# Chemical118/TREW

Hardware: AMD Instinct MI355X
Metric: Gbases/s scanned (short 5 32, 150 bp reads) (higher is better)
Workload: dtype u32

## Files before the change

include/trew_hip.h:

```cpp
#ifndef TREW_HIP_H
#define TREW_HIP_H

#include <stddef.h>
#include <stdint.h>

#ifdef __cplusplus
extern "C" {
#endif

#define TREW_HIP_ABI_VERSION 4

enum {
    TREW_MODE_SHORT = 0,
    TREW_MODE_PAIR = 1,
    TREW_MODE_LONG = 2,
    TREW_MODE_SEGMENT = 3
};

enum {
    TREW_TABLE_FORWARD_HIGH = 0,
    TREW_TABLE_FORWARD_LOW = 1,
    TREW_TABLE_BACKWARD_HIGH = 2,
    TREW_TABLE_BACKWARD_LOW = 3,
    TREW_TABLE_BOTH_HIGH = 4,
    TREW_TABLE_BOTH_LOW = 5,
    TREW_NUM_TABLES = 6
};

enum {
    TREW_FLAG_NO_FILTER = 1,
    TREW_FLAG_DEBUG_NO_EMIT = 2,
    TREW_FLAG_DEBUG_NO_KLOOP = 4,
    TREW_FLAG_DEBUG_POISON_LDS = 32,
    TREW_FLAG_DEBUG_WIDE_NO_WAIT = 128,
    TREW_FLAG_NO_TIMING = 64,
    TREW_FLAG_COMPAT_G1 = 512,
    TREW_FLAG_DEBUG_NO_JOINT = 2048,
    TREW_FLAG_DEBUG_NO_UNI_DRAIN = 4096,
    TREW_FLAG_DEBUG_NO_GROUP = 1024,
    TREW_FLAG_DEBUG_ANNOT_GENERAL = 8192,
    TREW_FLAG_TRACK_PRESSURE = 256
};

typedef struct {
    int32_t min_mer;
    int32_t max_mer;
    double low_baseline;
    double high_baseline;
    int32_t slice_length;
    int32_t mode;
    int32_t device;
    int32_t n_slots;
    uint64_t max_batch_words;
    uint64_t max_batch_reads;
    uint32_t table_log2_slots;
    uint32_t flags;
    uint64_t max_batch_ascii_bytes;
} trew_hip_params;

typedef struct {
    const uint32_t *words;
// ... 116 lines not shown
```

trew_amd/__init__.py:

```python
from . import capi
from .capi import (
    FLAG_NO_FILTER,
    FLAG_DEBUG_ANNOT_GENERAL,
    FLAG_DEBUG_POISON_LDS,
    FLAG_NO_TIMING,
    FLAG_TRACK_PRESSURE,
    FLAG_COMPAT_G1,
    FLAG_DEBUG_NO_GROUP,
    FLAG_DEBUG_NO_JOINT,
    FLAG_DEBUG_NO_UNI_DRAIN,
    FLAG_DEBUG_WIDE_NO_WAIT,
    MODE_LONG,
    MODE_PAIR,
    MODE_SEGMENT,
    MODE_SHORT,
    TABLE_NAMES,
    TrewHip,
    TrewHipError,
    annotate,
    k_mer_check,
    pack_reads,
)
```

trew_amd/capi.py:

```python
from __future__ import annotations

import ctypes as C
import os

import numpy as np

_HERE = os.path.dirname(os.path.abspath(__file__))
LIB_PATH = os.environ.get("TREW_HIP_LIB") or os.path.join(_HERE, "lib", "libtrew_hip.so")

MODE_SHORT, MODE_PAIR, MODE_LONG, MODE_SEGMENT = 0, 1, 2, 3
FLAG_NO_FILTER = 1
FLAG_DEBUG_POISON_LDS = 32
FLAG_NO_TIMING = 64
FLAG_COMPAT_G1 = 512
FLAG_TRACK_PRESSURE = 256
FLAG_DEBUG_NO_JOINT = 2048
FLAG_DEBUG_NO_UNI_DRAIN = 4096
FLAG_DEBUG_NO_GROUP = 1024
FLAG_DEBUG_ANNOT_GENERAL = 8192
FLAG_DEBUG_WIDE_NO_WAIT = 128
TABLE_NAMES = ("forward_high", "forward_low", "backward_high", "backward_low", "both_high", "both_low")

EXPORTED_SYMBOLS = (
    "trew_hip_init", "trew_hip_destroy", "trew_hip_last_error", "trew_hip_submit", "trew_hip_wait",
    "trew_hip_collect", "trew_hip_reset_tables", "trew_hip_add_rows", "trew_hip_segment_results",
    "trew_hip_filter_masks", "trew_hip_last_timing", "trew_pack_words", "trew_pack_reads",
    "trew_synth_short_ascii", "trew_synth_short_device", "trew_synth_pair_ascii", "trew_synth_pair_device",
    "trew_hip_malloc", "trew_hip_free", "trew_hip_memcpy_h2d", "trew_hip_memcpy_d2h", "trew_hip_abi_version",
    "trew_pack_pairs", "trew_hip_host_alloc", "trew_hip_host_free", "trew_hip_device_count",
    "trew_synth_long_lengths", "trew_synth_long_ascii", "trew_synth_long_device",
    "trew_hip_collect_device", "trew_hip_add_rows_device", "trew_hip_merge", "trew_hip_table_pressure",
    "trew_hip_add_gathered_device", "trew_hip_collect_slice_device", "trew_hip_debug_counters", "trew_hip_debug_worklist", "trew_hip_submit_ascii", "trew_hip_pack_ascii",
    "trew_motif_parse", "trew_hip_annotate", "trew_hip_annotate_results", "trew_annotate_host",
)
DEBUG_COUNTERS = ("strict_rerun", "windows_fallback", "wide_spin_timeout", "inserted", "inserted_wide", "group_punt", "group_routed", "group_target")


class Params(C.Structure):
    _fields_ = [
        ("min_mer", C.c_int32), ("max_mer", C.c_int32),
# ... 483 lines not shown
```

trew_amd/csrc/kernels/prefilter.inc:

```


template <int NW>
__device__ __forceinline__ void prefix_parity(const u32 (&f)[NW], u32 (&P)[NW]) {
    u32 carry = 0, prev_top = 0;
#pragma unroll
    for (int j = 0; j < NW; j++) {
        u32 x = f[j];
        x ^= x << 1;
        x ^= x << 2;
        x ^= x << 4;
        x ^= x << 8;
        x ^= x << 16;
        x ^= carry;
        P[j] = (x << 1) | prev_top;
        prev_top = x >> 31;
        carry = 0u - prev_top;
    }
}

template <>
__device__ __forceinline__ void prefix_parity<3>(const u32 (&f)[3], u32 (&P)[3]) {
    u64 x = ((u64) f[1] << 32) | f[0];
    x ^= x << 1;
    x ^= x << 2;
// ... 413 lines not shown
        const u32 lm = bits >= 32 ? 0xffffffffu : (bits <= 0 ? 0u : ((1u << bits) - 1u));
        f1[j] = lo[j] & lm;
        f2[j] = hi[j] & lm;
    }
    prefix_parity<3>(f1, o.P1);
    prefix_parity<3>(f2, o.P2);
}
__device__ __forceinline__ u32 bcnt_acc_s(u32 x, int acc) {
    u32 d;
    asm("v_bcnt_u32_b32 %0, %1, %2" : "=v"(d) : "v"(x), "s"(acc));
    return d;
}
__device__ __forceinline__ void halves_signs(u32 F1a, u32 F2a, u32 F1b, u32 F2b, int n2, int n1, int K, u32 &x, u32 &t) {
    u32 a = bcnt_acc_s(F1a, n2);
    u32 b = bcnt_acc_s(F2a, n2);
    u32 c = bcnt_acc_s(F1a & F2a, n1);
    a = bcnt_acc(F1b, a);
    b = bcnt_acc(F2b, b);
    c = bcnt_acc(F1b & F2b, c);
    const u32 p = a - c, q = b - c;
    x = __builtin_amdgcn_bitop3_b32(p, q, c, 0x80);
    t = a + q + (u32) K;
}
__device__ __forceinline__ u64 halves_verdict(u32 xA, u32 tA, u32 xB, u32 tB) {
    const u32 y = __builtin_amdgcn_bitop3_b32(xA, xB, tA, 0x40);
    const u32 z = __builtin_amdgcn_bitop3_b32(y, tB, tB, 0x30);
    return __ballot((int) z >= 0);
}
struct Thr8 {
    int4 a, b;
};
__device__ __forceinline__ Thr8 load_thr8(const int4 *p) {
    typedef int v8i __attribute__((ext_vector_type(8)));
    typedef const __attribute__((address_space(4))) v8i *cptr;
    const v8i v = *(cptr) (unsigned long long) p;
    Thr8 o;
    o.a = make_int4(v[0], v[1], v[2], v[3]);
    o.b = make_int4(v[4], v[5], v[6], v[7]);
    return o;
}
__device__ __forceinline__ int4 load_thr4(const int4 *p) {
    typedef int v4i __attribute__((ext_vector_type(4)));
    typedef const __attribute__((address_space(4))) v4i *cptr;
    const v4i v = *(cptr) (unsigned long long) p;
    return make_int4(v.x, v.y, v.z, v.w);
}

__device__ __forceinline__ const int4 *joint_thresholds(const int2 *thr_tab) { return (const int4 *) (thr_tab + kThrRows * kThrRow); }

__device__ __forceinline__ u64 filter_halves_uni(const HalvesP &A, const HalvesP &Bh, int L, int klo, int khi, const int4 *__restrict__ thr_row,
                                                 const u32 *wm_tab) {
    u64 trig = 0;
    int k = klo;
    const int4 *tp = thr_row + (klo - 1);
    {
        int b = L - 64;
        b = b > khi ? khi : b;
        auto probe = [&](u32 bs, const int4 t) __attribute__((always_inline)) -> u64 {
            u32 xA, tA, xB, tB;
            halves_signs(A.P1[0] ^ alignbit(A.P1[1], A.P1[0], bs), A.P2[0] ^ alignbit(A.P2[1], A.P2[0], bs), A.P1[1] ^ alignbit(A.P1[2], A.P1[1], bs),
                         A.P2[1] ^ alignbit(A.P2[2], A.P2[1], bs), t.x, t.y, t.z, xA, tA);
            halves_signs(Bh.P1[0] ^ alignbit(Bh.P1[1], Bh.P1[0], bs), Bh.P2[0] ^ alignbit(Bh.P2[1], Bh.P2[0], bs), Bh.P1[1] ^ alignbit(Bh.P1[2], Bh.P1[1], bs),
                         Bh.P2[1] ^ alignbit(Bh.P2[2], Bh.P2[1], bs), t.x, t.y, t.z, xB, tB);
            return halves_verdict(xA, tA, xB, tB);
        };
        for (; k + 1 <= b; k += 2, tp += 2) {
            const Thr8 t8 = load_thr8(tp);
            trig |= probe((u32) k, t8.a);
            trig |= probe((u32) k + 1u, t8.b);
        }
        if (k <= b) {
            trig |= probe((u32) k, load_thr4(tp));
            k++, tp++;
        }
    }
    if (k <= khi) {
        const int b = khi;
        const int s = L > 63 ? L - 63 : 0;
        const u64 QA1 = container64(A.P1, s), QA2 = container64(A.P2, s), QB1 = container64(Bh.P1, s), QB2 = container64(Bh.P2, s);
        u32 sh = (u32) (k - s);
        typedef const __attribute__((address_space(3))) u32 *lds_u32;
        u32 wa = (u32) (unsigned long long) (lds_u32) wm_tab + 4u * (u32) (63 - (L - k));
        asm volatile("" : "+v"(wa));
        auto probe = [&](u32 shk, u32 wmk, const int4 t) __attribute__((always_inline)) -> u64 {
            const u64 SA1 = QA1 >> shk, SA2 = QA2 >> shk, SB1 = QB1 >> shk, SB2 = QB2 >> shk;
            const u32 gA1 = xor_and(A.P1[1], (u32) (SA1 >> 32), wmk), gA2 = xor_and(A.P2[1], (u32) (SA2 >> 32), wmk);
            const u32 gB1 = xor_and(Bh.P1[1], (u32) (SB1 >> 32), wmk), gB2 = xor_and(Bh.P2[1], (u32) (SB2 >> 32), wmk);
            u32 xA, tA, xB, tB;
            halves_signs(A.P1[0] ^ (u32) SA1, A.P2[0] ^ (u32) SA2, gA1, gA2, t.x, t.y, t.z, xA, tA);
            halves_signs(Bh.P1[0] ^ (u32) SB1, Bh.P2[0] ^ (u32) SB2, gB1, gB2, t.x, t.y, t.z, xB, tB);
            return halves_verdict(xA, tA, xB, tB);
        };
        for (; k + 1 <= b; k += 2, sh += 2u, wa += 8u, tp += 2) {
            const Thr8 t8 = load_thr8(tp);
            const u32 wm0 = *(lds_u32) (unsigned long long) wa, wm1 = *(lds_u32) (unsigned long long) (wa + 4u);
            trig |= probe(sh, wm0, t8.a);
            trig |= probe(sh + 1u, wm1, t8.b);
        }
        if (k <= b) trig |= probe(sh, *(lds_u32) (unsigned long long) wa, load_thr4(tp));
    }
    return trig;
}

constexpr int kCntThr = 97;
__device__ __forceinline__ int4 count_thresholds(int c, float lowf) {
    const float prod = __fmul_rn((float) c, lowf);
    const int ithr = (int) floorf(prod) + 1;
    return make_int4(-2 * ithr, -ithr, 4 * ithr - c - 1, ithr);
}

struct DrainHalf {
    u32 P1[3], P2[3], P3[3];
    u32 V[3];
};
__device__ __forceinline__ void drain_half_init(const u32 (&lo)[3], const u32 (&hi)[3], const u32 (&nm)[3], int L, bool active, DrainHalf &h) {
    u32 f1[3], f2[3], f3[3];
#pragma unroll
    for (int j = 0; j < 3; j++) {
        const int bits = L - 32 * j;
        const u32 lm = bits >= 32 ? 0xffffffffu : (bits <= 0 ? 0u : ((1u << bits) - 1u));
        h.V[j] = active ? ~nm[j] & lm : 0u;
        f1[j] = lo[j] & lm;
        f2[j] = hi[j] & lm;
        f3[j] = f1[j] & f2[j];
// ... 18 lines not shown
    }
    const u32 p = a - c, q = b - c;
    const u32 t = a + q + (u32) th.z;
    return (int) __builtin_amdgcn_bitop3_b32(__builtin_amdgcn_bitop3_b32(p, q, c, 0x80), t, t, 0x30);
}
template <int N>
__device__ __forceinline__ bool drain_pass8(const u32 (&F1)[N], const u32 (&F2)[N], const u32 (&F3)[N], const u32 (&V)[N], u32 count, int ithr) {
    u32 c001 = 0, c010 = 0, c011 = 0, c100 = 0, c101 = 0, c110 = 0, c111 = 0;
#pragma unroll
    for (int j = 0; j < N; j++) {
        const u32 a11 = F1[j] & F2[j], a10 = F1[j] & ~F2[j], a01 = ~F1[j] & F2[j], a00 = V[j] & ~(F1[j] | F2[j]);
        const u32 b111 = a11 & F3[j], b101 = a10 & F3[j], b011 = a01 & F3[j], b001 = a00 & F3[j];
        c111 += __popc(b111);
        c110 += __popc(a11 ^ b111);
        c101 += __popc(b101);
        c100 += __popc(a10 ^ b101);
        c011 += __popc(b011);
        c010 += __popc(a01 ^ b011);
        c001 += __popc(b001);
    }
    const u32 c000 = count - c001 - c010 - c011 - c100 - c101 - c110 - c111;
    const u32 m8 = max(max(max(c000, c001), max(c010, c011)), max(max(c100, c101), max(c110, c111)));
    return (int) m8 >= ithr;
}

__device__ __forceinline__ bool drain_uni_applies(const DevParams &P, u32 UL, int gmax_run) {
    const int n_halves = P.mode == TREW_MODE_PAIR ? 4 : (P.mode == TREW_MODE_SHORT ? 2 : 0);
    if (n_halves == 0) return false;
    for (int slot = n_halves; slot < mode_slots(P.mode); slot++)
        if (get_segment(P.mode, slot, UL, UL, P.min_mer, P.max_mer, P.slice_len).valid) return false;
    for (int p = 0; p < n_halves; p += 2) {
        const Segment a = get_segment(P.mode, p, UL, UL, P.min_mer, P.max_mer, P.slice_len);
        const Segment b = get_segment(P.mode, p + 1, UL, UL, P.min_mer, P.max_mer, P.slice_len);
        const int la = (int) a.len, lb = (int) b.len, lmin = la < lb ? la : lb, lmax = la < lb ? lb : la;
        const int khi = a.kmax < gmax_run ? a.kmax : gmax_run;
        if (!(a.valid && b.valid && a.kmin == b.kmin && a.kmax == b.kmax && lmax <= 95 && lmax - lmin <= 1 && a.kmin >= 1 && khi <= lmin)) return false;
    }
    return true;
}

__device__ __forceinline__ bool filter_deferred_uni(const DevParams &P, const DevBatch &B, u64 unit, bool active, int gmax_run,
                                                    const int4 *cnt_thr) {
    const u32 UL = B.uniform_length;
    ReadRef rd[2];
    rd[0].w = B.words;
    rd[0].len = 0;
// ... 10 lines not shown
    const u64 actm = __ballot(active);
    u64 flag = 0;
    const int n_halves = P.mode == TREW_MODE_PAIR ? 4 : 2;
    for (int p = 0; p < n_halves && flag != actm; p += 2) {
        const Segment sA = get_segment(P.mode, p, UL, UL, P.min_mer, P.max_mer, P.slice_len);
        const Segment sB = get_segment(P.mode, p + 1, UL, UL, P.min_mer, P.max_mer, P.slice_len);
        const int LA = rfl_i((int) sA.len), LB = rfl_i((int) sB.len), Lmax = LA < LB ? LB : LA;
        const int klo = rfl_i(sA.kmin > P.min_mer ? sA.kmin : P.min_mer), khi = rfl_i(sA.kmax < gmax_run ? sA.kmax : gmax_run);
        DrainHalf A, Bh;
        {
            u32 lo[3], hi[3], nm[3];
            load_planes<3>(sA.mate ? rd[1] : rd[0], sA.start, lo, hi, nm);
            drain_half_init(lo, hi, nm, LA, active, A);
            load_planes<3>(sB.mate ? rd[1] : rd[0], sB.start, lo, hi, nm);
            drain_half_init(lo, hi, nm, LB, active, Bh);
        }
        for (int t = 1; t < klo; t++) {
            drain_v_step3(A.V);
            drain_v_step3(Bh.V);
        }
        int k = klo;
        {
            const int b = khi < Lmax - 64 ? khi : Lmax - 64;
            auto half3 = [&](const DrainHalf &h, u32 bs) __attribute__((always_inline)) -> u64 {
                const u32 cnt = bcnt_acc(h.V[2], bcnt_acc(h.V[1], __popc(h.V[0])));
                const int4 th = cnt_thr[cnt];
                u32 F1[3], F2[3];
#pragma unroll
                for (int j = 0; j < 3; j++) {
                    F1[j] = xor_and(h.P1[j], alignbit(j < 2 ? h.P1[j < 2 ? j + 1 : 0] : 0u, h.P1[j], bs), h.V[j]);
                    F2[j] = xor_and(h.P2[j], alignbit(j < 2 ? h.P2[j < 2 ? j + 1 : 0] : 0u, h.P2[j], bs), h.V[j]);
                }
                const u64 p4 = __ballot(drain_signs<3>(F1, F2, th) >= 0);
                u64 p8 = 0;
                if (p4 & ~flag) {
                    u32 F3[3];
#pragma unroll
                    for (int j = 0; j < 3; j++) F3[j] = h.P3[j] ^ alignbit(j < 2 ? h.P3[j < 2 ? j + 1 : 0] : 0u, h.P3[j], bs);
                    p8 = __ballot(drain_pass8<3>(F1, F2, F3, h.V, cnt, th.w));
                }
                return p8;
            };
            for (; k <= b && flag != actm; k++) {
                flag |= half3(A, (u32) k);
                flag |= half3(Bh, (u32) k);
                drain_v_step3(A.V);
                drain_v_step3(Bh.V);
            }
        }
        if (k <= khi && flag != actm) {
            const int oA = LA > 63 ? LA - 63 : 0, oB = LB > 63 ? LB - 63 : 0;
            const u64 QA1 = container64(A.P1, oA), QA2 = container64(A.P2, oA), QB1 = container64(Bh.P1, oB), QB2 = container64(Bh.P2, oB);
            u64 VA = ((u64) A.V[1] << 32) | A.V[0], VB = ((u64) Bh.V[1] << 32) | Bh.V[0];
            auto half2 = [&](const DrainHalf &h, u64 Q1, u64 Q2, u64 V, int s) __attribute__((always_inline)) -> u64 {
                const u32 v0 = (u32) V, v1 = (u32) (V >> 32);
                const u32 cnt = bcnt_acc(v1, __popc(v0));
                const int4 th = cnt_thr[cnt];
                const u32 sh = (u32) (k - s);
                const u64 S1 = Q1 >> sh, S2 = Q2 >> sh;
                const u32 F1[2] = {xor_and(h.P1[0], (u32) S1, v0), xor_and(h.P1[1], (u32) (S1 >> 32), v1)};
                const u32 F2[2] = {xor_and(h.P2[0], (u32) S2, v0), xor_and(h.P2[1], (u32) (S2 >> 32), v1)};
                const u64 p4 = __ballot(drain_signs<2>(F1, F2, th) >= 0);
                u64 p8 = 0;
                if (p4 & ~flag) {
                    const u64 S3 = container64(h.P3, s) >> sh;
                    const u32 F3[2] = {h.P3[0] ^ (u32) S3, h.P3[1] ^ (u32) (S3 >> 32)};
                    const u32 Vw[2] = {v0, v1};
                    p8 = __ballot(drain_pass8<2>(F1, F2, F3, Vw, cnt, th.w));
                }
                return p8;
            };
            for (; k <= khi && flag != actm; k++) {
                flag |= half2(A, QA1, QA2, VA, oA);
                flag |= half2(Bh, QB1, QB2, VB, oB);
                VA &= VA >> 1;
                VB &= VB >> 1;
            }
        }
    }
    return (flag >> lane_id()) & 1ull;
}

constexpr u32 kFilterThreads = TREW_FILTER_THREADS;
constexpr u32 kStage = kFilterThreads == 256 ? 1024 : 192;
constexpr u32 kDefer = 2 * kFilterThreads;

template <int NW>
#ifndef TREW_FILTER3_WAVES
#define TREW_FILTER3_WAVES 6
#endif
#ifndef TREW_FILTER5_WAVES
#define TREW_FILTER5_WAVES 6
#endif
__global__ __launch_bounds__(kFilterThreads, (NW <= 3 ? TREW_FILTER3_WAVES : (NW == 5 ? TREW_FILTER5_WAVES : 1))) void filter_kernel(DevParams P, DevBatch B, u32 *wl, u32 *wl_count, u32 wl_cap,
                                                                u64 *dbg_masks, int dbg_slots, int max_seg, u32 *diag,
                                                                const int2 *__restrict__ thr_tab) {
#ifdef TREW_AB_FILTER_PRIO
    __builtin_amdgcn_s_setprio(TREW_AB_FILTER_PRIO);
#endif
    __shared__ u32 stage[kStage];
    __shared__ u32 stage_n, flush_base;
    __shared__ u32 defer_n;
    u32 defer_seen = 0;
    if (threadIdx.x == 0) stage_n = 0;
    __syncthreads();
    auto flush = [&]() __attribute__((always_inline)) {
        const u32 n = stage_n;
        if (n) {
// ... 59 lines not shown
#pragma unroll
                        for (int j = 0; j < NW; j++) {
                            lo[j] = hi[j] = 0;
                            nm[j] = 0xffffffffu;
                        }
                    }
                    u64 m;
                    if (P.flags & TREW_FLAG_NO_FILTER)
                        m = all_k_mask(sg.kmin, sg.kmax);
                    else
                        m = filter_segment<NW>(lo, hi, nm, ok ? (int) sg.len : 0, sg.kmin, sg.kmax, P.min_mer, gmax_run, max_seg, P.lowf);
                    mask = ok ? m : 0ull;
                }
                if (active && sg.valid && sg.len > (u32) (32 * NW - 1)) mask = all_k_mask(sg.kmin, sg.kmax);
                any |= mask;
                if (dbg_masks && active && slot < dbg_slots) dbg_masks[unit * (u64) dbg_slots + slot] = mask;
            }
        }
        return any;
    };

    __shared__ u32 defer[kDefer];
    __shared__ unsigned char defer_kind[kDefer];
    __shared__ u32 wm_tab[34];
    if (threadIdx.x < 34) wm_tab[threadIdx.x] = threadIdx.x < 32 ? 0xffffffffu >> threadIdx.x : 0u;
    __shared__ int4 cnt_thr[kCntThr];
    for (u32 i = threadIdx.x; i < (u32) kCntThr; i += blockDim.x) cnt_thr[i] = count_thresholds((int) i, P.lowf);
    const u32 UL = B.uniform_length;
    const bool uni = NW <= 5 && UL != 0 && thr_tab != nullptr && P.mode != TREW_MODE_LONG && !(P.flags & TREW_FLAG_NO_FILTER);
    const bool uni_drain = NW == 3 && uni && !dbg_masks && !(P.flags & TREW_FLAG_DEBUG_NO_UNI_DRAIN) && drain_uni_applies(P, UL, gmax_run);
    if (threadIdx.x == 0) defer_n = 0;
    __syncthreads();
    __shared__ u32 next_chunk[2];
    constexpr u32 kChunkShards = 8;
    const u32 my_shard = blockIdx.x & (kChunkShards - 1u);
    auto shard_ctr = [&](u32 sh) __attribute__((always_inline)) { return wl_count + 32u + 32u * sh + kChunkCounterWord; };
    u64 chunk = blockIdx.x;
    u32 round = 0;
    for (;;) {
        const bool more = chunk * kFilterThreads < B.n_units;
        if (more) {
            const u64 unit = chunk * kFilterThreads + threadIdx.x;
            const bool active = unit < B.n_units;
            u32 nxt = 0;
#ifndef TREW_AB_STATIC_CHUNKS
            if (threadIdx.x == 0) nxt = gridDim.x + kChunkShards * atomicAdd(shard_ctr(my_shard), 1u) + my_shard;
#else
            nxt = (u32) chunk + gridDim.x;
#endif
            u64 any = 0;
            bool dfr = active, dfr_n = false;
            if constexpr (NW <= 5) {
                if (uni) {
                    ReadRef rd[2];
                    rd[0].w = B.words;
                    rd[0].len = 0;
                    rd[0].nw = 0;
                    rd[1] = rd[0];
                    if (active) {
                        if (P.mode == TREW_MODE_PAIR) {
                            rd[0] = get_read(B, 2 * unit);
                            rd[1] = get_read(B, 2 * unit + 1);
                        } else {
                            rd[0] = get_read(B, unit);
                        }
                    }
                    dfr = false;
                    int slot0 = 0;
#ifndef TREW_AB_NO_JOINT
                    if constexpr (NW == 3) {
                        const int n_halves = P.mode == TREW_MODE_PAIR ? 4 : (P.mode == TREW_MODE_SHORT ? 2 : 0);
                        for (; slot0 + 1 < n_halves && !dbg_masks && !(P.flags & TREW_FLAG_DEBUG_NO_JOINT); slot0 += 2) {
                            const Segment sA = get_segment(P.mode, slot0, UL, UL, P.min_mer, P.max_mer, P.slice_len);
                            const Segment sB = get_segment(P.mode, slot0 + 1, UL, UL, P.min_mer, P.max_mer, P.slice_len);
                            const int L = rfl_i((int) sA.len);
                            const int klo = rfl_i(sA.kmin > P.min_mer ? sA.kmin : P.min_mer), khi = rfl_i(sA.kmax < gmax_run ? sA.kmax : gmax_run);
                            const bool uneq = sB.len == sA.len + 1u;
                            if (!(sA.valid && sB.valid && (sA.len == sB.len || uneq) && sA.len <= 95u && sA.kmin == sB.kmin && sA.kmax == sB.kmax &&
                                  klo >= L + 1 - kUniSubsetMax && khi <= L - 32 && klo <= 31))
                                break;
                            u32 loA[3], hiA[3], nmA[3], loB[3], hiB[3], nmB[3];
                            load_planes<3>(sA.mate ? rd[1] : rd[0], sA.start, loA, hiA, nmA);
                            load_planes<3>(sB.mate ? rd[1] : rd[0], sB.start, loB, hiB, nmB);
                            u32 anyn = 0;
#pragma unroll
                            for (int j = 0; j < 3; j++) {
                                const int bits = L - 32 * j, bitsB = (int) sB.len - 32 * j;
                                const u32 lm = bits >= 32 ? 0xffffffffu : (bits <= 0 ? 0u : ((1u << bits) - 1u));
                                const u32 lmB = bitsB >= 32 ? 0xffffffffu : (bitsB <= 0 ? 0u : ((1u << bitsB) - 1u));
                                anyn |= (nmA[j] & lm) | (nmB[j] & lmB);
                            }
                            dfr = dfr || (active && anyn != 0);
                            dfr_n = dfr_n || (active && anyn != 0);
                            HalvesP hA, hB;
                            halves_prefix(loA, hiA, L, hA);
                            halves_prefix(loB, hiB, L, hB);
                            const u64 trig = filter_halves_uni(hA, hB, L, klo, khi, joint_thresholds(thr_tab) + (uneq ? 2 + slot0 / 2 : slot0 / 2) * kThrRow, wm_tab);
                            dfr = dfr || (active && any == 0 && ((trig >> lane_id()) & 1ull) != 0);
                        }
                    }
#endif
                    for (int slot = slot0; slot < nslots; slot++) {
                        const Segment sg = get_segment(P.mode, slot, UL, UL, P.min_mer, P.max_mer, P.slice_len);
                        if (!sg.valid) continue;
                        if (sg.len > (u32) (32 * NW - 1)) {
                            dfr = dfr || active;
                            continue;
                        }
                        u32 lo[NW], hi[NW], nm[NW];
                        const ReadRef r = sg.mate ? rd[1] : rd[0];
                        load_planes<NW>(r, sg.start, lo, hi, nm);
                        u32 anyn = 0;
#pragma unroll
                        for (int j = 0; j < NW; j++) {
                            const int bits = (int) sg.len - 32 * j;
                            const u32 lm = bits >= 32 ? 0xffffffffu : (bits <= 0 ? 0u : ((1u << bits) - 1u));
                            anyn |= nm[j] & lm;
                        }
                        UniVerdict vd;
                        filter_segment_uni<NW>(lo, hi, (int) sg.len, sg.kmin, sg.kmax, P.min_mer, gmax_run, thr_tab + slot * kThrRow, dbg_masks != nullptr, vd);
                        dfr = dfr || (active && anyn != 0);
                        dfr_n = dfr_n || (active && anyn != 0);
                        any |= (vd.flagm >> lane_id()) & 1ull;
                        if (dbg_masks && active && anyn == 0 && slot < dbg_slots)
                            dbg_masks[unit * (u64) dbg_slots + slot] = ((((u64) vd.chi) << 32) | vd.clo) & all_k_mask(sg.kmin, sg.kmax);
                    }
                }
            }
            {
                const u64 bal = __ballot(dfr);
                if (bal) {
                    const u32 lane = lane_id();
                    const int leader = __ffsll((long long) bal) - 1;
                    u32 sb = 0;
                    if ((int) lane == leader) sb = atomicAdd(&defer_n, (u32) __popcll(bal));
                    sb = __shfl(sb, leader);
                    if (dfr) {
                        const u32 at = sb + (u32) __popcll(bal & ((1ull << lane) - 1ull));
                        defer[at] = (u32) unit;
                        defer_kind[at] = dfr_n ? 1 : 0;
                    }
                }
            }
            if (threadIdx.x == 0) next_chunk[round & 1u] = nxt;
            append(active && !dfr && any != 0, (u32) unit);
            chunk = next_chunk[round & 1u];
#ifndef TREW_AB_STATIC_CHUNKS
            if (chunk * kFilterThreads >= B.n_units) {
                __syncthreads();
                if (threadIdx.x == 0) {
                    u64 c = chunk;
                    for (u32 att = 1; att < kChunkShards && c * kFilterThreads >= B.n_units; att++) {
                        const u32 sh = (my_shard + att) & (kChunkShards - 1u);
                        c = (u64) gridDim.x + (u64) kChunkShards * atomicAdd(shard_ctr(sh), 1u) + sh;
                    }
                    next_chunk[round & 1u] = (u32) (c < 0xffffffffull ? c : 0xffffffffull);
                }
                __syncthreads();
                chunk = next_chunk[round & 1u];
                __syncthreads();
            }
#endif
            round++;
        }
        const u32 dn = defer_seen;
        if (dn >= kFilterThreads || (!more && dn > 0u)) {
            const u32 take = dn < kFilterThreads ? dn : kFilterThreads;
            const u32 at = dn - take;
            const bool active2 = threadIdx.x < take;
            const u32 unit2 = active2 ? defer[at + threadIdx.x] : 0u;
            const bool n2 = active2 && defer_kind[at + threadIdx.x] != 0;
            __syncthreads();
            if (threadIdx.x == 0) defer_n = at;
#ifndef TREW_AB_SKIP_DRAIN
            const u64 any2 = uni_drain ? (u64) filter_deferred_uni(P, B, unit2, active2, gmax_run, cnt_thr) : general(unit2, active2);
#else
            u64 any2 = 0;
            u32 keep = unit2;
            asm volatile("" : "+v"(keep), "+v"(any2));
            (void) keep;
#endif
            append(active2 && any2 != 0 && !n2, unit2);
            append(active2 && any2 != 0 && n2, unit2);
        } else if (!more) {
            break;
        }
    }
    flush();
}
```

trew_amd/csrc/trew_capi.cpp:

```cpp
#include <hip/hip_runtime.h>

#include <algorithm>
#include <atomic>
#include <cmath>
#include <cstdio>
#include <cstdlib>
#include <cstring>
#include <mutex>
#include <string>
#include <thread>
#include <vector>

#include "trew_common.hpp"
#include "trew_launch.hpp"
#include "trew_synth.hpp"

using namespace trew;

namespace {

struct Slot {
    hipStream_t stream = nullptr;
    u32 *d_buf = nullptr;
    u32 *d_words = nullptr, *d_offsets = nullptr, *d_lengths = nullptr;
// ... 932 lines not shown
}

extern "C" int trew_hip_debug_worklist(trew_hip_ctx *ctx, int slot, uint32_t *units, uint64_t cap, uint64_t *n) {
    if (!ctx || !n) return -1;
    if (slot < 0 || slot >= (int) ctx->slots.size()) return fail(ctx, "slot out of range");
    HIPCHK(ctx, hipSetDevice(ctx->p.device));
    Slot &s = ctx->slots[(size_t) slot];
    HIPCHK(ctx, hipStreamSynchronize(s.stream));
    u32 c = 0;
    if (s.n_launches) HIPCHK(ctx, hipMemcpy(&c, s.d_wl_count + ((s.n_launches - 1) & 1) * kWlCountWords, 4, hipMemcpyDeviceToHost));
    c = (u32) std::min<u64>(c, ctx->p.max_batch_reads);
    *n = c;
    const u64 take = std::min<u64>(c, cap);
    if (units && take) HIPCHK(ctx, hipMemcpy(units, s.d_wl, take * 4, hipMemcpyDeviceToHost));
    return 0;
}

extern "C" int trew_hip_debug_counters(trew_hip_ctx *ctx, uint64_t *out, int n) {
    if (!ctx || !out || n < 0) return -1;
    if (int rc = sync_all(ctx)) return rc;
    u32 diag[kDiagWords], fb[kFallbackWords];
    HIPCHK(ctx, hipMemcpy(diag, ctx->table.overflow, sizeof(diag), hipMemcpyDeviceToHost));
    HIPCHK(ctx, fallback_counters_read(fb));
    const u32 v[TREW_DEBUG_COUNTERS] = {fb[kFallbackStrictRerun], fb[kFallbackWindows], fb[kFallbackWideSpin], diag[kDiagInserted], diag[kDiagInsertedWide], fb[kFallbackGroupPunt], fb[kFallbackGroupRouted], fb[kFallbackGroupTarget]};
    for (int i = 0; i < n; i++) out[i] = i < TREW_DEBUG_COUNTERS ? v[i] : 0;
    return 0;
}

extern "C" int trew_hip_merge(trew_hip_ctx *dst, trew_hip_ctx *src) {
    if (!dst || !src) return -1;
    if (dst == src) return fail(dst, "trew_hip_merge: source and destination are the same context");
    std::mutex *m1 = &dst->table_mu, *m2 = &src->table_mu;
    if (m2 < m1) std::swap(m1, m2);
    std::lock_guard<std::mutex> l1(*m1), l2(*m2);
    if (int rc = sync_all(src)) return rc;
    u64 n = 0;
    if (int rc = compact_to(src, -1, nullptr, 0, &n)) return rc;
    if (n == 0) return 0;
    if (int rc = ensure_rows(src, &src->d_collect_rows, &src->collect_cap, n)) return rc;
    if (int rc = compact_to(src, -1, src->d_collect_rows, src->collect_cap, &n)) return rc;
    if (int rc = sync_all(dst)) return rc;
    if (int rc = ensure_rows(dst, &dst->d_add_rows, &dst->add_cap, n)) return rc;
    HIPCHK(dst, hipSetDevice(dst->p.device));
    HIPCHK(dst, hipMemcpyPeerAsync(dst->d_add_rows, dst->p.device, src->d_collect_rows, src->p.device, n * sizeof(trew_hip_row), dst->slots[0].stream));
    return add_device_rows_locked(dst, dst->d_add_rows, n, false);
}
// ... 542 lines not shown
```

trew_amd/csrc/trew_kernels.hip:

```cpp
#include <hip/hip_runtime.h>

#include <algorithm>
#include <cstdlib>

#include "trew_common.hpp"
#include "trew_launch.hpp"
#include "trew_synth.hpp"

#ifndef TREW_FILTER_THREADS
#define TREW_FILTER_THREADS 256
#endif

namespace trew {

typedef unsigned __int128 u128;

#include "kernels/helpers.inc"
#include "kernels/prefilter.inc"
#include "kernels/count_table.inc"
#include "kernels/exact_core.inc"
#include "kernels/decide_group.inc"
#include "kernels/driver_long.inc"
#include "kernels/driver_pair.inc"
#include "kernels/exact_kernel.inc"
// ... 62 lines not shown
    }
}

hipError_t launch_filter(hipStream_t st, u32 n_cu, u32 max_seg_len, const DevParams &P, const DevBatch &B, u32 *wl, u32 *wl_count,
                         u32 wl_cap, u64 *dbg_masks, int dbg_slots, u32 *diag, const int2 *d_thr) {
    const int nw = pick_nw(max_seg_len);
    const int max_seg = (int) std::min<u32>(max_seg_len, (u32) (32 * nw - 1));
    if (B.n_units == 0) return hipSuccess;
    typedef void (*kern_t)(DevParams, DevBatch, u32 *, u32 *, u32, u64 *, int, int, u32 *, const int2 *);
    const kern_t fn = nw == 3 ? filter_kernel<3> : nw == 5 ? filter_kernel<5> : nw == 10 ? filter_kernel<10> : filter_kernel<32>;
    const u32 threads = kFilterThreads;
    static thread_local kern_t cached_fn = nullptr;
    static thread_local int cached_per_cu = 0;
    int per_cu = cached_per_cu;
    if (cached_fn != fn) {
        if (hipOccupancyMaxActiveBlocksPerMultiprocessor(&per_cu, (const void *) fn, (int) threads, 0) != hipSuccess || per_cu < 1) per_cu = 4;
        if (const char *e = getenv("TREW_FILTER_BLOCKS_PER_CU")) per_cu = std::max(1, atoi(e));
        cached_fn = fn;
        cached_per_cu = per_cu;
    }
    u64 blocks = (B.n_units + threads - 1) / threads;
    const u64 persistent = (u64) n_cu * (u64) per_cu;
    if (blocks > persistent) blocks = persistent;
    hipLaunchKernelGGL(fn, dim3((u32) blocks), dim3(threads), 0, st, P, B, wl, wl_count, wl_cap, dbg_masks, dbg_slots, max_seg, diag, d_thr);
    return hipGetLastError();
}

hipError_t fallback_counters_read(u32 *out) { return hipMemcpyFromSymbol(out, HIP_SYMBOL(g_fallback), sizeof(u32) * kFallbackWords); }
hipError_t fallback_counters_clear(hipStream_t st) {
    void *p = nullptr;
    const hipError_t e = hipGetSymbolAddress(&p, HIP_SYMBOL(g_fallback));
    return e != hipSuccess ? e : hipMemsetAsync(p, 0, sizeof(u32) * kFallbackWords, st);
}

u32 exact_lds_bytes_host(u32 cap, u32 rawwords, u32 wordbytes) { return exact_lds_bytes(cap, rawwords, wordbytes); }

hipError_t launch_g1_apply(hipStream_t st, const DevTable &T, const DevG1 &G, const DevBatch &B, int min_mer, const trew_hip_row *carry_in,
                           trew_hip_row *carry_out, u32 carry_cap) {
    hipLaunchKernelGGL(g1_apply_kernel, dim3(256), dim3(256), 0, st, T, G, B, min_mer, carry_in, carry_out, carry_cap);
    hipLaunchKernelGGL(g1_finish_kernel, dim3(1), dim3(1), 0, st, G);
    return hipGetLastError();
}

hipError_t launch_exact(hipStream_t st, u32 n_cu, u64 n_units, const DevParams &P, const DevBatch &B, const DevTableG1 &T,
                        const u32 *wl, u32 *wl_count, u32 *wl_count_next, u32 wl_cap, const SegResults &R, u32 cap, u32 rawwords,
                        u32 max_seg_len, bool share) {
// ... 126 lines not shown
```

Baseline: 1994.

## Defer individual triggered halves instead of whole reads in the uniform drain

The joint prefilter now keeps separate verdict accumulators for each half, so only the halves that triggered are pushed to the defer queue. The drain then re-checks each half on its own thread and ORs sibling verdicts through shared memory. The goal is to avoid re-scanning both halves of a read when only one is suspicious, and to spread drain work across more lanes. In exchange the defer buffer grows from 2x to 5x the thread count, a per-thread verdict array and extra barriers are added, and queue cuts must be aligned to head items. The ballot is moved out of the inner probe loop, which also removes per-k wave reductions.

```diff
diff --git a/include/trew_hip.h b/include/trew_hip.h
--- a/include/trew_hip.h
+++ b/include/trew_hip.h
@@ -37,6 +37,7 @@
     TREW_FLAG_COMPAT_G1 = 512,
     TREW_FLAG_DEBUG_NO_JOINT = 2048,
     TREW_FLAG_DEBUG_NO_UNI_DRAIN = 4096,
+    TREW_FLAG_DEBUG_READ_DRAIN = 16384,
     TREW_FLAG_DEBUG_NO_GROUP = 1024,
     TREW_FLAG_DEBUG_ANNOT_GENERAL = 8192,
     TREW_FLAG_TRACK_PRESSURE = 256
diff --git a/trew_amd/__init__.py b/trew_amd/__init__.py
--- a/trew_amd/__init__.py
+++ b/trew_amd/__init__.py
@@ -9,6 +9,7 @@
     FLAG_DEBUG_NO_GROUP,
     FLAG_DEBUG_NO_JOINT,
     FLAG_DEBUG_NO_UNI_DRAIN,
+    FLAG_DEBUG_READ_DRAIN,
     FLAG_DEBUG_WIDE_NO_WAIT,
     MODE_LONG,
     MODE_PAIR,
diff --git a/trew_amd/capi.py b/trew_amd/capi.py
--- a/trew_amd/capi.py
+++ b/trew_amd/capi.py
@@ -16,6 +16,7 @@
 FLAG_TRACK_PRESSURE = 256
 FLAG_DEBUG_NO_JOINT = 2048
 FLAG_DEBUG_NO_UNI_DRAIN = 4096
+FLAG_DEBUG_READ_DRAIN = 16384
 FLAG_DEBUG_NO_GROUP = 1024
 FLAG_DEBUG_ANNOT_GENERAL = 8192
 FLAG_DEBUG_WIDE_NO_WAIT = 128
diff --git a/trew_amd/csrc/kernels/prefilter.inc b/trew_amd/csrc/kernels/prefilter.inc
--- a/trew_amd/csrc/kernels/prefilter.inc
+++ b/trew_amd/csrc/kernels/prefilter.inc
@@ -459,11 +459,7 @@
     x = __builtin_amdgcn_bitop3_b32(p, q, c, 0x80);
     t = a + q + (u32) K;
 }
-__device__ __forceinline__ u64 halves_verdict(u32 xA, u32 tA, u32 xB, u32 tB) {
-    const u32 y = __builtin_amdgcn_bitop3_b32(xA, xB, tA, 0x40);
-    const u32 z = __builtin_amdgcn_bitop3_b32(y, tB, tB, 0x30);
-    return __ballot((int) z >= 0);
-}
+__device__ __forceinline__ u32 half_acc(u32 acc, u32 x, u32 t) { return __builtin_amdgcn_bitop3_b32(acc, x, t, 0x40); }
 struct Thr8 {
     int4 a, b;
 };
@@ -485,29 +481,30 @@
 
 __device__ __forceinline__ const int4 *joint_thresholds(const int2 *thr_tab) { return (const int4 *) (thr_tab + kThrRows * kThrRow); }
 
-__device__ __forceinline__ u64 filter_halves_uni(const HalvesP &A, const HalvesP &Bh, int L, int klo, int khi, const int4 *__restrict__ thr_row,
-                                                 const u32 *wm_tab) {
-    u64 trig = 0;
+__device__ __forceinline__ void filter_halves_uni(const HalvesP &A, const HalvesP &Bh, int L, int klo, int khi, const int4 *__restrict__ thr_row,
+                                                  const u32 *wm_tab, u32 &accA, u32 &accB) {
+    accA = accB = 0xffffffffu;
     int k = klo;
     const int4 *tp = thr_row + (klo - 1);
     {
         int b = L - 64;
         b = b > khi ? khi : b;
-        auto probe = [&](u32 bs, const int4 t) __attribute__((always_inline)) -> u64 {
+        auto probe = [&](u32 bs, const int4 t) __attribute__((always_inline)) {
             u32 xA, tA, xB, tB;
             halves_signs(A.P1[0] ^ alignbit(A.P1[1], A.P1[0], bs), A.P2[0] ^ alignbit(A.P2[1], A.P2[0], bs), A.P1[1] ^ alignbit(A.P1[2], A.P1[1], bs),
                          A.P2[1] ^ alignbit(A.P2[2], A.P2[1], bs), t.x, t.y, t.z, xA, tA);
             halves_signs(Bh.P1[0] ^ alignbit(Bh.P1[1], Bh.P1[0], bs), Bh.P2[0] ^ alignbit(Bh.P2[1], Bh.P2[0], bs), Bh.P1[1] ^ alignbit(Bh.P1[2], Bh.P1[1], bs),
                          Bh.P2[1] ^ alignbit(Bh.P2[2], Bh.P2[1], bs), t.x, t.y, t.z, xB, tB);
-            return halves_verdict(xA, tA, xB, tB);
+            accA = half_acc(accA, xA, tA);
+            accB = half_acc(accB, xB, tB);
         };
         for (; k + 1 <= b; k += 2, tp += 2) {
             const Thr8 t8 = load_thr8(tp);
-            trig |= probe((u32) k, t8.a);
-            trig |= probe((u32) k + 1u, t8.b);
+            probe((u32) k, t8.a);
+            probe((u32) k + 1u, t8.b);
         }
         if (k <= b) {
-            trig |= probe((u32) k, load_thr4(tp));
+            probe((u32) k, load_thr4(tp));
             k++, tp++;
         }
     }
@@ -519,24 +516,24 @@
         typedef const __attribute__((address_space(3))) u32 *lds_u32;
         u32 wa = (u32) (unsigned long long) (lds_u32) wm_tab + 4u * (u32) (63 - (L - k));
         asm volatile("" : "+v"(wa));
-        auto probe = [&](u32 shk, u32 wmk, const int4 t) __attribute__((always_inline)) -> u64 {
+        auto probe = [&](u32 shk, u32 wmk, const int4 t) __attribute__((always_inline)) {
             const u64 SA1 = QA1 >> shk, SA2 = QA2 >> shk, SB1 = QB1 >> shk, SB2 = QB2 >> shk;
             const u32 gA1 = xor_and(A.P1[1], (u32) (SA1 >> 32), wmk), gA2 = xor_and(A.P2[1], (u32) (SA2 >> 32), wmk);
             const u32 gB1 = xor_and(Bh.P1[1], (u32) (SB1 >> 32), wmk), gB2 = xor_and(Bh.P2[1], (u32) (SB2 >> 32), wmk);
             u32 xA, tA, xB, tB;
             halves_signs(A.P1[0] ^ (u32) SA1, A.P2[0] ^ (u32) SA2, gA1, gA2, t.x, t.y, t.z, xA, tA);
             halves_signs(Bh.P1[0] ^ (u32) SB1, Bh.P2[0] ^ (u32) SB2, gB1, gB2, t.x, t.y, t.z, xB, tB);
-            return halves_verdict(xA, tA, xB, tB);
+            accA = half_acc(accA, xA, tA);
+            accB = half_acc(accB, xB, tB);
         };
         for (; k + 1 <= b; k += 2, sh += 2u, wa += 8u, tp += 2) {
             const Thr8 t8 = load_thr8(tp);
             const u32 wm0 = *(lds_u32) (unsigned long long) wa, wm1 = *(lds_u32) (unsigned long long) (wa + 4u);
-            trig |= probe(sh, wm0, t8.a);
-            trig |= probe(sh + 1u, wm1, t8.b);
-        }
-        if (k <= b) trig |= probe(sh, *(lds_u32) (unsigned long long) wa, load_thr4(tp));
-    }
-    return trig;
+            probe(sh, wm0, t8.a);
+            probe(sh + 1u, wm1, t8.b);
+        }
+        if (k <= b) probe(sh, *(lds_u32) (unsigned long long) wa, load_thr4(tp));
+    }
 }
 
 constexpr int kCntThr = 97;
@@ -601,6 +598,48 @@
     const u32 c000 = count - c001 - c010 - c011 - c100 - c101 - c110 - c111;
     const u32 m8 = max(max(max(c000, c001), max(c010, c011)), max(max(c100, c101), max(c110, c111)));
     return (int) m8 >= ithr;
+}
+
+__device__ __forceinline__ u64 drain_probe3(const DrainHalf &h, u32 bs, const int4 *cnt_thr, u64 flag) {
+    const u32 cnt = bcnt_acc(h.V[2], bcnt_acc(h.V[1], __popc(h.V[0])));
+    const int4 th = cnt_thr[cnt];
+    u32 F1[3], F2[3];
+#pragma unroll
+    for (int j = 0; j < 3; j++) {
+        F1[j] = xor_and(h.P1[j], alignbit(j < 2 ? h.P1[j < 2 ? j + 1 : 0] : 0u, h.P1[j], bs), h.V[j]);
+        F2[j] = xor_and(h.P2[j], alignbit(j < 2 ? h.P2[j < 2 ? j + 1 : 0] : 0u, h.P2[j], bs), h.V[j]);
+    }
+    const u64 p4 = __ballot(drain_signs<3>(F1, F2, th) >= 0);
+    u64 p8 = 0;
+    if (p4 & ~flag) {
+        u32 F3[3];
+#pragma unroll
+        for (int j = 0; j < 3; j++) F3[j] = h.P3[j] ^ alignbit(j < 2 ? h.P3[j < 2 ? j + 1 : 0] : 0u, h.P3[j], bs);
+        p8 = __ballot(drain_pass8<3>(F1, F2, F3, h.V, cnt, th.w));
+    }
+    return p8;
+}
+__device__ __forceinline__ u64 drain_probe2(const DrainHalf &h, u64 Q1, u64 Q2, u64 V, int s, u32 sh, const int4 *cnt_thr, u64 flag) {
+    const u32 v0 = (u32) V, v1 = (u32) (V >> 32);
+    const u32 cnt = bcnt_acc(v1, __popc(v0));
+    const int4 th = cnt_thr[cnt];
+    const u64 S1 = Q1 >> sh, S2 = Q2 >> sh;
+    const u32 F1[2] = {xor_and(h.P1[0], (u32) S1, v0), xor_and(h.P1[1], (u32) (S1 >> 32), v1)};
+    const u32 F2[2] = {xor_and(h.P2[0], (u32) S2, v0), xor_and(h.P2[1], (u32) (S2 >> 32), v1)};
+    const u64 p4 = __ballot(drain_signs<2>(F1, F2, th) >= 0);
+    u64 p8 = 0;
+    if (p4 & ~flag) {
+        const u64 S3 = container64(h.P3, s) >> sh;
+        const u32 F3[2] = {h.P3[0] ^ (u32) S3, h.P3[1] ^ (u32) (S3 >> 32)};
+        const u32 Vw[2] = {v0, v1};
+        p8 = __ballot(drain_pass8<2>(F1, F2, F3, Vw, cnt, th.w));
+    }
+    return p8;
+}
+
+__device__ __forceinline__ bool joint_applies(const Segment &sA, const Segment &sB, int L, int klo, int khi) {
+    return sA.valid && sB.valid && (sA.len == sB.len || sB.len == sA.len + 1u) && sA.len <= 95u && sA.kmin == sB.kmin && sA.kmax == sB.kmax &&
+           klo >= L + 1 - kUniSubsetMax && khi <= L - 32 && klo <= 31;
 }
 
 __device__ __forceinline__ bool drain_uni_applies(const DevParams &P, u32 UL, int gmax_run) {
@@ -657,28 +696,9 @@
         int k = klo;
         {
             const int b = khi < Lmax - 64 ? khi : Lmax - 64;
-            auto half3 = [&](const DrainHalf &h, u32 bs) __attribute__((always_inline)) -> u64 {
-                const u32 cnt = bcnt_acc(h.V[2], bcnt_acc(h.V[1], __popc(h.V[0])));
-                const int4 th = cnt_thr[cnt];
-                u32 F1[3], F2[3];
-#pragma unroll
-                for (int j = 0; j < 3; j++) {
-                    F1[j] = xor_and(h.P1[j], alignbit(j < 2 ? h.P1[j < 2 ? j + 1 : 0] : 0u, h.P1[j], bs), h.V[j]);
-                    F2[j] = xor_and(h.P2[j], alignbit(j < 2 ? h.P2[j < 2 ? j + 1 : 0] : 0u, h.P2[j], bs), h.V[j]);
-                }
-                const u64 p4 = __ballot(drain_signs<3>(F1, F2, th) >= 0);
-                u64 p8 = 0;
-                if (p4 & ~flag) {
-                    u32 F3[3];
-#pragma unroll
-                    for (int j = 0; j < 3; j++) F3[j] = h.P3[j] ^ alignbit(j < 2 ? h.P3[j < 2 ? j + 1 : 0] : 0u, h.P3[j], bs);
-                    p8 = __ballot(drain_pass8<3>(F1, F2, F3, h.V, cnt, th.w));
-                }
-                return p8;
-            };
             for (; k <= b && flag != actm; k++) {
-                flag |= half3(A, (u32) k);
-                flag |= half3(Bh, (u32) k);
+                flag |= drain_probe3(A, (u32) k, cnt_thr, flag);
+                flag |= drain_probe3(Bh, (u32) k, cnt_thr, flag);
                 drain_v_step3(A.V);
                 drain_v_step3(Bh.V);
             }
@@ -687,27 +707,9 @@
             const int oA = LA > 63 ? LA - 63 : 0, oB = LB > 63 ? LB - 63 : 0;
             const u64 QA1 = container64(A.P1, oA), QA2 = container64(A.P2, oA), QB1 = container64(Bh.P1, oB), QB2 = container64(Bh.P2, oB);
             u64 VA = ((u64) A.V[1] << 32) | A.V[0], VB = ((u64) Bh.V[1] << 32) | Bh.V[0];
-            auto half2 = [&](const DrainHalf &h, u64 Q1, u64 Q2, u64 V, int s) __attribute__((always_inline)) -> u64 {
-                const u32 v0 = (u32) V, v1 = (u32) (V >> 32);
-                const u32 cnt = bcnt_acc(v1, __popc(v0));
-                const int4 th = cnt_thr[cnt];
-                const u32 sh = (u32) (k - s);
-                const u64 S1 = Q1 >> sh, S2 = Q2 >> sh;
-                const u32 F1[2] = {xor_and(h.P1[0], (u32) S1, v0), xor_and(h.P1[1], (u32) (S1 >> 32), v1)};
-                const u32 F2[2] = {xor_and(h.P2[0], (u32) S2, v0), xor_and(h.P2[1], (u32) (S2 >> 32), v1)};
-                const u64 p4 = __ballot(drain_signs<2>(F1, F2, th) >= 0);
-                u64 p8 = 0;
-                if (p4 & ~flag) {
-                    const u64 S3 = container64(h.P3, s) >> sh;
-                    const u32 F3[2] = {h.P3[0] ^ (u32) S3, h.P3[1] ^ (u32) (S3 >> 32)};
-                    const u32 Vw[2] = {v0, v1};
-                    p8 = __ballot(drain_pass8<2>(F1, F2, F3, Vw, cnt, th.w));
-                }
-                return p8;
-            };
             for (; k <= khi && flag != actm; k++) {
-                flag |= half2(A, QA1, QA2, VA, oA);
-                flag |= half2(Bh, QB1, QB2, VB, oB);
+                flag |= drain_probe2(A, QA1, QA2, VA, oA, (u32) (k - oA), cnt_thr, flag);
+                flag |= drain_probe2(Bh, QB1, QB2, VB, oB, (u32) (k - oB), cnt_thr, flag);
                 VA &= VA >> 1;
                 VB &= VB >> 1;
             }
@@ -716,9 +718,70 @@
     return (flag >> lane_id()) & 1ull;
 }
 
+constexpr u32 kItemN = 1u, kItemHead = 2u, kItemHalfShift = 2u, kItemSibShift = 4u;
+
+__device__ __forceinline__ bool drain_half_applies(const DevParams &P, u32 UL, int gmax_run) {
+    if (!drain_uni_applies(P, UL, gmax_run) || (P.flags & TREW_FLAG_DEBUG_NO_JOINT)) return false;
+    const int n_halves = P.mode == TREW_MODE_PAIR ? 4 : 2;
+    const Segment a = get_segment(P.mode, 0, UL, UL, P.min_mer, P.max_mer, P.slice_len);
+    const int L = (int) a.len, klo = a.kmin > P.min_mer ? a.kmin : P.min_mer, khi = a.kmax < gmax_run ? a.kmax : gmax_run;
+    for (int h = 0; h < n_halves; h += 2) {
+        const Segment b = get_segment(P.mode, h, UL, UL, P.min_mer, P.max_mer, P.slice_len);
+        const Segment c = get_segment(P.mode, h + 1, UL, UL, P.min_mer, P.max_mer, P.slice_len);
+        if (b.len != a.len || c.len != a.len || b.kmin != a.kmin || b.kmax != a.kmax) return false;
+        if (!joint_applies(b, c, L, klo, khi)) return false;
+    }
+    return true;
+}
+
+__device__ __forceinline__ bool filter_deferred_half(const DevParams &P, const DevBatch &B, u32 unit, u32 half, bool active, int gmax_run,
+                                                     const int4 *cnt_thr) {
+    const u32 UL = B.uniform_length;
+    const bool pair = P.mode == TREW_MODE_PAIR;
+    const int n_halves = pair ? 4 : 2;
+    const Segment s0 = get_segment(P.mode, 0, UL, UL, P.min_mer, P.max_mer, P.slice_len);
+    u32 start = s0.start, mate = s0.mate;
+    for (int h = 1; h < n_halves; h++) {
+        const Segment sh = get_segment(P.mode, h, UL, UL, P.min_mer, P.max_mer, P.slice_len);
+        start = half == (u32) h ? sh.start : start;
+        mate = half == (u32) h ? sh.mate : mate;
+    }
+    const int L = rfl_i((int) s0.len);
+    const int klo = rfl_i(s0.kmin > P.min_mer ? s0.kmin : P.min_mer), khi = rfl_i(s0.kmax < gmax_run ? s0.kmax : gmax_run);
+    ReadRef rd;
+    rd.w = B.words;
+    rd.len = 0;
+    rd.nw = 0;
+    if (active) rd = get_read(B, pair ? 2 * (u64) unit + mate : (u64) unit);
+    DrainHalf A;
+    {
+        u32 lo[3], hi[3], nm[3];
+        load_planes<3>(rd, start, lo, hi, nm);
+        drain_half_init(lo, hi, nm, L, active, A);
+    }
+    for (int t = 1; t < klo; t++) drain_v_step3(A.V);
+    const u64 actm = __ballot(active);
+    u64 flag = 0;
+    int k = klo;
+    for (const int b = khi < L - 64 ? khi : L - 64; k <= b && flag != actm; k++) {
+        flag |= drain_probe3(A, (u32) k, cnt_thr, flag);
+        drain_v_step3(A.V);
+    }
+    if (k <= khi && flag != actm) {
+        const int o = L > 63 ? L - 63 : 0;
+        const u64 Q1 = container64(A.P1, o), Q2 = container64(A.P2, o);
+        u64 V = ((u64) A.V[1] << 32) | A.V[0];
+        for (; k <= khi && flag != actm; k++) {
+            flag |= drain_probe2(A, Q1, Q2, V, o, (u32) (k - o), cnt_thr, flag);
+            V &= V >> 1;
+        }
+    }
+    return (flag >> lane_id()) & 1ull;
+}
+
 constexpr u32 kFilterThreads = TREW_FILTER_THREADS;
 constexpr u32 kStage = kFilterThreads == 256 ? 1024 : 192;
-constexpr u32 kDefer = 2 * kFilterThreads;
+constexpr u32 kDefer = 5 * kFilterThreads;
 
 template <int NW>
 #ifndef TREW_FILTER3_WAVES
@@ -824,6 +887,7 @@
 
     __shared__ u32 defer[kDefer];
     __shared__ unsigned char defer_kind[kDefer];
+    __shared__ unsigned char verdict[kFilterThreads];
     __shared__ u32 wm_tab[34];
     if (threadIdx.x < 34) wm_tab[threadIdx.x] = threadIdx.x < 32 ? 0xffffffffu >> threadIdx.x : 0u;
     __shared__ int4 cnt_thr[kCntThr];
@@ -831,6 +895,11 @@
     const u32 UL = B.uniform_length;
     const bool uni = NW <= 5 && UL != 0 && thr_tab != nullptr && P.mode != TREW_MODE_LONG && !(P.flags & TREW_FLAG_NO_FILTER);
     const bool uni_drain = NW == 3 && uni && !dbg_masks && !(P.flags & TREW_FLAG_DEBUG_NO_UNI_DRAIN) && drain_uni_applies(P, UL, gmax_run);
+#ifndef TREW_AB_NO_JOINT
+    const bool half_drain = uni_drain && !(P.flags & TREW_FLAG_DEBUG_READ_DRAIN) && drain_half_applies(P, UL, gmax_run);
+#else
+    const bool half_drain = false;
+#endif
     if (threadIdx.x == 0) defer_n = 0;
     __syncthreads();
     __shared__ u32 next_chunk[2];
@@ -852,6 +921,7 @@
 #endif
             u64 any = 0;
             bool dfr = active, dfr_n = false;
+            u32 items = 0;
             if constexpr (NW <= 5) {
                 if (uni) {
                     ReadRef rd[2];
@@ -878,27 +948,28 @@
                             const int L = rfl_i((int) sA.len);
                             const int klo = rfl_i(sA.kmin > P.min_mer ? sA.kmin : P.min_mer), khi = rfl_i(sA.kmax < gmax_run ? sA.kmax : gmax_run);
                             const bool uneq = sB.len == sA.len + 1u;
-                            if (!(sA.valid && sB.valid && (sA.len == sB.len || uneq) && sA.len <= 95u && sA.kmin == sB.kmin && sA.kmax == sB.kmax &&
-                                  klo >= L + 1 - kUniSubsetMax && khi <= L - 32 && klo <= 31))
-                                break;
+                            if (!joint_applies(sA, sB, L, klo, khi)) break;
                             u32 loA[3], hiA[3], nmA[3], loB[3], hiB[3], nmB[3];
                             load_planes<3>(sA.mate ? rd[1] : rd[0], sA.start, loA, hiA, nmA);
                             load_planes<3>(sB.mate ? rd[1] : rd[0], sB.start, loB, hiB, nmB);
-                            u32 anyn = 0;
+                            u32 anynA = 0, anynB = 0;
 #pragma unroll
                             for (int j = 0; j < 3; j++) {
                                 const int bits = L - 32 * j, bitsB = (int) sB.len - 32 * j;
                                 const u32 lm = bits >= 32 ? 0xffffffffu : (bits <= 0 ? 0u : ((1u << bits) - 1u));
                                 const u32 lmB = bitsB >= 32 ? 0xffffffffu : (bitsB <= 0 ? 0u : ((1u << bitsB) - 1u));
-                                anyn |= (nmA[j] & lm) | (nmB[j] & lmB);
+                                anynA |= nmA[j] & lm;
+                                anynB |= nmB[j] & lmB;
                             }
-                            dfr = dfr || (active && anyn != 0);
-                            dfr_n = dfr_n || (active && anyn != 0);
                             HalvesP hA, hB;
                             halves_prefix(loA, hiA, L, hA);
                             halves_prefix(loB, hiB, L, hB);
-                            const u64 trig = filter_halves_uni(hA, hB, L, klo, khi, joint_thresholds(thr_tab) + (uneq ? 2 + slot0 / 2 : slot0 / 2) * kThrRow, wm_tab);
-                            dfr = dfr || (active && any == 0 && ((trig >> lane_id()) & 1ull) != 0);
+                            u32 accA, accB;
+                            filter_halves_uni(hA, hB, L, klo, khi, joint_thresholds(thr_tab) + (uneq ? 2 + slot0 / 2 : slot0 / 2) * kThrRow, wm_tab, accA, accB);
+                            const bool itA = active && (anynA != 0 || (int) accA >= 0), itB = active && (anynB != 0 || (int) accB >= 0);
+                            items |= ((itA ? 1u : 0u) | (itB ? 2u : 0u)) << slot0;
+                            dfr_n = dfr_n || (active && (anynA | anynB) != 0);
+                            dfr = dfr || itA || itB;
                         }
                     }
 #endif
@@ -929,7 +1000,43 @@
                     }
                 }
             }
+#ifdef TREW_AB_COUNT_ITEMS
             {
+                const u32 w_units = (u32) __popcll(__ballot(dfr)), w_items = wave_sum_u32((u32) __popc(items));
+                const u32 w_n = (u32) __popcll(__ballot(dfr_n));
+                if (lane_id() == 0) {
+                    atomicAdd(&diag[8], w_units);
+                    atomicAdd(&diag[9], w_items);
+                    atomicAdd(&diag[11], w_n);
+                }
+            }
+#endif
+            if (NW == 3 && half_drain) {
+                const u32 lane = lane_id();
+                const u64 below = (1ull << lane) - 1ull;
+                const int n_halves = P.mode == TREW_MODE_PAIR ? 4 : 2;
+                u32 off = 0, tot = 0;
+                for (int h = 0; h < n_halves; h++) {
+                    const u64 bal = __ballot(((items >> h) & 1u) != 0);
+                    off += (u32) __popcll(bal & below);
+                    tot += (u32) __popcll(bal);
+                }
+                if (tot) {
+                    u32 sb = 0;
+                    if (lane == 0) sb = atomicAdd(&defer_n, tot);
+                    u32 at = __shfl(sb, 0) + off;
+                    const u32 common = (dfr_n ? kItemN : 0u) | (((u32) __popc(items) - 1u) << kItemSibShift);
+                    u32 head = kItemHead;
+                    for (int h = 0; h < n_halves; h++) {
+                        if ((items >> h) & 1u) {
+                            defer[at] = (u32) unit;
+                            defer_kind[at] = (unsigned char) (common | head | ((u32) h << kItemHalfShift));
+                            at++;
+                            head = 0;
+                        }
+                    }
+                }
+            } else {
                 const u64 bal = __ballot(dfr);
                 if (bal) {
                     const u32 lane = lane_id();
@@ -940,7 +1047,7 @@
                     if (dfr) {
                         const u32 at = sb + (u32) __popcll(bal & ((1ull << lane) - 1ull));
                         defer[at] = (u32) unit;
-                        defer_kind[at] = dfr_n ? 1 : 0;
+                        defer_kind[at] = dfr_n ? kItemN : 0;
                     }
                 }
             }
@@ -965,28 +1072,47 @@
 #endif
             round++;
         }
-        const u32 dn = defer_seen;
-        if (dn >= kFilterThreads || (!more && dn > 0u)) {
-            const u32 take = dn < kFilterThreads ? dn : kFilterThreads;
-            const u32 at = dn - take;
+        for (;;) {
+            const u32 dn = defer_seen;
+            if (!(dn >= kFilterThreads || (!more && dn > 0u))) break;
+            u32 at = dn < kFilterThreads ? 0u : dn - kFilterThreads;
+            if (NW == 3 && half_drain)
+                for (int i = 0; i < 3 && !(defer_kind[at] & kItemHead); i++) at++;
+#ifdef TREW_AB_COUNT_ITEMS
+            if (threadIdx.x == 0 && dn >= kFilterThreads && at != dn - kFilterThreads) atomicAdd(&diag[10], 1u);
+#endif
+            const u32 take = dn - at;
             const bool active2 = threadIdx.x < take;
             const u32 unit2 = active2 ? defer[at + threadIdx.x] : 0u;
-            const bool n2 = active2 && defer_kind[at + threadIdx.x] != 0;
+            const u32 kind2 = active2 ? (u32) defer_kind[at + threadIdx.x] : 0u;
+            const bool n2 = (kind2 & kItemN) != 0;
             __syncthreads();
             if (threadIdx.x == 0) defer_n = at;
 #ifndef TREW_AB_SKIP_DRAIN
-            const u64 any2 = uni_drain ? (u64) filter_deferred_uni(P, B, unit2, active2, gmax_run, cnt_thr) : general(unit2, active2);
+            bool any2;
+            if (NW == 3 && half_drain) {
+                verdict[threadIdx.x] = filter_deferred_half(P, B, unit2, (kind2 >> kItemHalfShift) & 3u, active2, gmax_run, cnt_thr) ? 1 : 0;
+                __syncthreads();
+                u32 v = 0;
+                if (kind2 & kItemHead) {
+                    const u32 sib = (kind2 >> kItemSibShift) & 3u;
+                    for (u32 i = 0; i <= sib; i++) v |= verdict[threadIdx.x + i];
+                }
+                any2 = v != 0;
+            } else {
+                any2 = (uni_drain ? (u64) filter_deferred_uni(P, B, unit2, active2, gmax_run, cnt_thr) : general(unit2, active2)) != 0;
+            }
 #else
-            u64 any2 = 0;
-            u32 keep = unit2;
-            asm volatile("" : "+v"(keep), "+v"(any2));
+            u32 any2v = 0;
+            u32 keep = unit2 ^ kind2;
+            asm volatile("" : "+v"(keep), "+v"(any2v));
             (void) keep;
-#endif
-            append(active2 && any2 != 0 && !n2, unit2);
-            append(active2 && any2 != 0 && n2, unit2);
-        } else if (!more) {
-            break;
-        }
+            const bool any2 = any2v != 0;
+#endif
+            append(active2 && any2 && !n2, unit2);
+            append(active2 && any2 && n2, unit2);
+        }
+        if (!more) break;
     }
     flush();
 }
diff --git a/trew_amd/csrc/trew_capi.cpp b/trew_amd/csrc/trew_capi.cpp
--- a/trew_amd/csrc/trew_capi.cpp
+++ b/trew_amd/csrc/trew_capi.cpp
@@ -978,6 +978,9 @@
     u32 diag[kDiagWords], fb[kFallbackWords];
     HIPCHK(ctx, hipMemcpy(diag, ctx->table.overflow, sizeof(diag), hipMemcpyDeviceToHost));
     HIPCHK(ctx, fallback_counters_read(fb));
+#ifdef TREW_AB_COUNT_ITEMS
+    fprintf(stderr, "TREW_AB_COUNT_ITEMS set_aside_units=%u half_items=%u cuts_moved=%u n_units=%u\n", diag[8], diag[9], diag[10], diag[11]);
+#endif
     const u32 v[TREW_DEBUG_COUNTERS] = {fb[kFallbackStrictRerun], fb[kFallbackWindows], fb[kFallbackWideSpin], diag[kDiagInserted], diag[kDiagInsertedWide], fb[kFallbackGroupPunt], fb[kFallbackGroupRouted], fb[kFallbackGroupTarget]};
     for (int i = 0; i < n; i++) out[i] = i < TREW_DEBUG_COUNTERS ? v[i] : 0;
     return 0;
diff --git a/trew_amd/csrc/trew_kernels.hip b/trew_amd/csrc/trew_kernels.hip
--- a/trew_amd/csrc/trew_kernels.hip
+++ b/trew_amd/csrc/trew_kernels.hip
@@ -108,6 +108,7 @@
     u64 blocks = (B.n_units + threads - 1) / threads;
     const u64 persistent = (u64) n_cu * (u64) per_cu;
     if (blocks > persistent) blocks = persistent;
+    if (const char *e = getenv("TREW_FILTER_MAX_BLOCKS")) blocks = std::min<u64>(blocks, (u64) std::max(1, atoi(e)));
     hipLaunchKernelGGL(fn, dim3((u32) blocks), dim3(threads), 0, st, P, B, wl, wl_count, wl_cap, dbg_masks, dbg_slots, max_seg, diag, d_thr);
     return hipGetLastError();
 }
```

New measurement: 2064 (median of 6 runs). 3.5% higher.
